# TencentEMapReduce/alluxio

Hardware: AMD Instinct MI355X
Metric: StressWorkerBench cached seq-read GB/s (whole node) at 1/2/4/8 MI355X workers (higher is better)
Workload: dtype uint8; 1 GPU; model=StressWorkerBench cached seq-read, HBM MEM tier, global_batch=256, seq_len=4096, parallelism=workers1, threads_per_worker=256, block_size=67108864, buffer_size=4096, page_size=2097152, verified=True, headline_verified=True, full=False

## Files before the change

### alluxio_amd/csrc/bindings.cpp

```cpp
#include <pybind11/pybind11.h>
#include <pybind11/stl.h>
#include <pybind11/numpy.h>

#include <cmath>
#include <cstring>
#include <vector>

#include "block_store.h"
#include "trace.h"
#include "cpu_codecs.h"
#include "ipc.h"
#include "numa_host.h"
#include "ring_read.h"
#include "ragged_gather.h"
#include "delim_index.h"
#include "field_parse.h"
#include "text_column.h"
#include "json_fields.h"
#include "parquet_decode.h"
#include "parquet_encode.h"
#include "parquet_stats.h"
#include "text_dict.h"
#include "kernels.h"
#include "seg_ring.h"
// ... 1144 lines not shown
          const size_t nc = (n + bpc - 1) / bpc;
          std::string out(nc * 4, '\0');
          {
            py::gil_scoped_release rel;
            for (size_t i = 0; i < nc; ++i) {
              const size_t off = i * bpc;
              const uint32_t c = crc32c_sw(p + off, std::min<size_t>(bpc, n - off), 0);
              out[4 * i] = char(c >> 24); out[4 * i + 1] = char(c >> 16);
              out[4 * i + 2] = char(c >> 8); out[4 * i + 3] = char(c);
            }
          }
          return py::bytes(out);
        }, py::arg("data"), py::arg("bytes_per_checksum") = 512);
  m.def("crc32c_combine", &crc32c_combine);
  m.def("crc32c_device_pages", &crc32c_device_pages, G(), py::arg("base"), py::arg("pages"), py::arg("length"),
        py::arg("page_bytes"));
  m.def("crc32c_device", &crc32c_device, G(), py::arg("ptr"), py::arg("length"), py::arg("piece") = 0,
        py::arg("stream") = 0);
  m.def("lz4_compress", [](py::bytes data) {
          std::string s = data;
          std::string out(lz4_compress_bound(s.size()), '\0');
          int64_t n;
          {
            py::gil_scoped_release rel;
            n = lz4_compress_block((const uint8_t*)s.data(), s.size(), (uint8_t*)&out[0], out.size());
          }
          if (n < 0) throw StoreError(kErrInvalidArgument, "lz4 compression failed");
          out.resize((size_t)n);
          return py::bytes(out);
        });
  m.def("lz4_decompress", [](py::bytes data, size_t capacity) {
          std::string s = data;
          std::string out(capacity, '\0');
          int64_t n;
          {
            py::gil_scoped_release rel;
            n = lz4_decompress_block((const uint8_t*)s.data(), s.size(), (uint8_t*)&out[0], out.size());
          }
          if (n < 0) throw StoreError(kErrInvalidArgument, "malformed lz4 block (" + std::to_string(n) + ")");
          out.resize((size_t)n);
          return py::bytes(out);
        });
  m.def("lz4_compress_bound", &lz4_compress_bound);
  m.def("trace_push", [](const std::string& name) { roctxRangePushA(name.c_str()); }, py::arg("name"));
  m.def("trace_pop", [] { roctxRangePop(); });
  m.def("trace_mark", [](const std::string& name) { roctxMarkA(name.c_str()); }, py::arg("name"));
  m.def("lz4_device", &lz4_device, G(), py::arg("chunks"), py::arg("compress"), py::arg("stream") = 0);
  m.def("lz4_device_kernel_ms", &lz4_device_kernel_ms, G(), py::arg("chunks"), py::arg("compress"),
        py::arg("reps") = 5);
  m.def("batched_copy", &batched_copy, G(), py::arg("segments"), py::arg("stream") = 0, py::arg("sync") = true);
  m.def("fill_pattern", [](uint64_t ptr, uint64_t bytes, uint64_t seed, uint64_t word_offset, uint64_t stream) {
          py::gil_scoped_release rel;
          HIP_CHECK(launch_fill_pattern(reinterpret_cast<uint8_t*>(ptr), bytes, seed, word_offset,
                                        reinterpret_cast<hipStream_t>(stream)));
        }, py::arg("ptr"), py::arg("bytes"), py::arg("seed"), py::arg("word_offset") = 0, py::arg("stream") = 0);
  m.def("store_fill", [](uint64_t ptr, uint64_t bytes, uint32_t word, bool nontemporal, unsigned grid,
                         uint64_t stream) {
          py::gil_scoped_release rel;
          unsigned used = 0;
          HIP_CHECK(launch_store_fill(reinterpret_cast<uint8_t*>(ptr), bytes, word, nontemporal, grid, &used,
                                      reinterpret_cast<hipStream_t>(stream)));
          return used;
        }, py::arg("ptr"), py::arg("bytes"), py::arg("word") = 0, py::arg("nontemporal") = false,
        py::arg("grid") = 0, py::arg("stream") = 0);
  m.def("evict_select_device", &evict_select_device);
  m.def("page_alloc_device", &page_alloc_device);
  m.def("set_copy_variant", &set_copy_variant, py::arg("variant"), py::arg("grid_cap") = 0);
  m.def("copy_variant", [] {
    int v = 0;
    unsigned cap = 0;
    copy_variant(&v, &cap);
    return py::make_tuple(v, cap);
  });
  m.def("set_crc_variant", &set_crc_variant, py::arg("variant"));
  m.def("set_lz4_decode_variant", &set_lz4_decode_variant, py::arg("variant"));
  m.def("set_lz4_encode_variant", &set_lz4_encode_variant, py::arg("variant"));
  m.def("set_seq_read_variant", &set_seq_read_variant, py::arg("variant"), py::arg("grid_cap") = 0);
  m.def("seq_read_variant", [] {
    int v = 0;
    unsigned cap = 0;
    seq_read_variant(&v, &cap);
    return py::make_tuple(v, cap);
  });
  m.def("seq_read_last_launch", [] {
    const SeqReadLaunch l = seq_read_last_launch();
    return py::make_tuple(l.fast ? "fast" : "general", l.unroll, l.grid);
  });
  m.def("set_ragged_gather_variant", &set_ragged_gather_variant, py::arg("variant"), py::arg("chunk_shift") = 0);
  m.def("ragged_gather_chunk_shift", &ragged_gather_chunk_shift);
  m.def("set_delim_index_variant", &set_delim_index_variant, py::arg("variant"), py::arg("tile_shift") = 0);
  m.def("delim_index_tile_shift", &delim_index_tile_shift);
  m.def("delim_index_variant", &delim_index_variant);
  m.def("set_delim_quote_variant", &set_delim_quote_variant, py::arg("variant"));
  m.def("delim_quote_variant", &delim_quote_variant);
  m.def("set_field_parse_variant", &set_field_parse_variant, py::arg("variant"));
  m.def("field_parse_variant", &field_parse_variant);
  m.def("set_text_column_variant", &set_text_column_variant, py::arg("variant"));
  m.def("text_column_variant", &text_column_variant);
  m.def("set_json_fields_variant", &set_json_fields_variant, py::arg("variant"));
  m.def("json_fields_variant", &json_fields_variant);
  m.def("set_json_text_variant", &set_json_text_variant, py::arg("variant"));
  m.def("json_text_variant", &json_text_variant);
  m.def("set_parquet_decode_variant", &set_parquet_decode_variant, py::arg("variant"));
  m.def("parquet_decode_variant", &parquet_decode_variant);
  m.def("set_text_dict_variant", &set_text_dict_variant, py::arg("variant"));
  m.def("text_dict_variant", &text_dict_variant);
  m.def("set_page_gather_chunk_variant", &set_page_gather_chunk_variant, py::arg("variant"));
  m.attr("COPY_CHUNK") = kCopyChunk;
}
```

### alluxio_amd/csrc/kernels.h

```cpp
#pragma once
#include <hip/hip_runtime.h>
#include <cstddef>
#include <cstdint>

#include "field_parse_host.h"
#include "json_fields_host.h"
#include "json_text_host.h"
#include "parquet_encode_host.h"
#include "parquet_host.h"
#include "parquet_stats_host.h"
#include "text_column_host.h"
#include "text_dict_host.h"

namespace amdx {

struct CopySeg {
  uint64_t src;
  uint64_t dst;
  uint64_t bytes;
  uint64_t chunk0;
};

constexpr uint64_t kCopyChunk = 256 * 1024;

hipError_t launch_batched_copy(const CopySeg* segs, int nseg, uint64_t total_chunks,
                               hipStream_t stream);
void set_copy_variant(int variant, unsigned grid_cap);
void copy_variant(int* variant, unsigned* grid_cap);

struct SeqReadArgs {
  const uint8_t* arena;
  const int64_t* ftab;
  const uint64_t* c_init;
  uint8_t* dst;
  uint64_t stream_stride;
  uint64_t file_len;
  uint64_t buf;
  uint64_t launch_base;
  uint32_t cycle;
  uint32_t streams;
  uint32_t depth;
  uint32_t page_shift;
  uint64_t footprint = 0;
  uint64_t base_mod = ~0ull;
};
constexpr uint32_t kSeqReadMaxStreams = 8192;
hipError_t launch_seq_read(const SeqReadArgs& a, hipStream_t stream);
void set_seq_read_variant(int variant, unsigned grid_cap);
void seq_read_variant(int* variant, unsigned* grid_cap);
struct SeqReadLaunch {
  int fast;
  int unroll;
  unsigned grid;
};
SeqReadLaunch seq_read_last_launch();
hipError_t launch_store_fill(uint8_t* dst, uint64_t bytes, uint32_t word, bool nontemporal, unsigned grid,
                             unsigned* grid_used, hipStream_t stream);

struct RaggedRow {
  uint64_t src;
  uint64_t dst_off;
  uint64_t span;
  uint32_t len;
  uint32_t chunk0;
};
struct RaggedRec {
  uint64_t start;
  uint32_t len;
  uint32_t pad;
};
struct RaggedGatherArgs {
  const uint8_t* arena;
  const int64_t* vtab;
  const RaggedRec* recs;
  const int64_t* idx;
  uint8_t* dst;
  uint64_t* out_off;
  uint32_t* out_len;
  RaggedRow* rows;
  uint32_t* chunk_pre;
  uint64_t n_rec;
  uint64_t row_stride;
  uint32_t batch;
  uint32_t page_shift;
  uint32_t align;
  uint32_t max_len;
  uint32_t padded;
  uint32_t pad_value;
  uint32_t total_chunks;
  uint32_t chunk_shift;
};
constexpr uint32_t kRaggedGatherMaxBatch = 65536;
hipError_t launch_ragged_gather(const RaggedGatherArgs& a, hipStream_t stream);
void set_ragged_gather_variant(int variant, unsigned chunk_shift);
uint32_t ragged_gather_chunk_shift();

struct DelimIndexArgs {
  const uint8_t* arena;
  const int64_t* vtab;
  uint32_t* tile_count;
  uint64_t* tile_base;
  uint64_t* out;
  uint64_t out_cap;
  uint64_t vstart;
  uint64_t bytes;
  uint64_t add;
  uint32_t ntiles;
  uint32_t page_shift;
  uint32_t tile_shift;
  uint32_t delim;
  uint32_t quote;
  uint32_t in_quote;
  uint32_t* tile_count_odd;
  uint32_t* tile_parity;
};
uint64_t delim_index_tiles(uint64_t vstart, uint64_t bytes, uint32_t tile_shift);
hipError_t launch_delim_count(const DelimIndexArgs& a, hipStream_t stream);
hipError_t launch_delim_scan(const DelimIndexArgs& a, hipStream_t stream);
hipError_t launch_delim_emit(const DelimIndexArgs& a, uint64_t total, hipStream_t stream);
hipError_t launch_delim_count_quoted(const DelimIndexArgs& a, hipStream_t stream);
hipError_t launch_delim_scan_quoted(const DelimIndexArgs& a, hipStream_t stream);
hipError_t launch_delim_emit_quoted(const DelimIndexArgs& a, uint64_t total, hipStream_t stream);
void set_delim_quote_variant(int variant);
int delim_quote_variant();
void set_delim_index_variant(int variant, unsigned tile_shift);
uint32_t delim_index_tile_shift();
int delim_index_variant();

hipError_t launch_field_parse(const FieldParseArgs& a, hipStream_t stream);
void set_field_parse_variant(int variant);
int field_parse_variant();

hipError_t launch_text_measure(const TextColumnArgs& a, hipStream_t stream);
hipError_t launch_text_emit(const TextColumnArgs& a, hipStream_t stream);
void set_text_column_variant(int variant);
int text_column_variant();
// ... 195 lines not shown
```

### alluxio_amd/csrc/kernels.hip

```cpp
#include "kernels.h"

#include <algorithm>
#include <cstring>
#include <mutex>

namespace amdx {

constexpr int kCopyThreads = 256;
typedef unsigned int u32x4 __attribute__((ext_vector_type(4)));

template <int P>
__device__ __forceinline__ u32x4 ld16(const u32x4* p) {
  if constexpr (P == 1) return __builtin_nontemporal_load(p);
  else return *p;
}
template <int P>
__device__ __forceinline__ void st16(u32x4* p, u32x4 v) {
  if constexpr (P == 1) __builtin_nontemporal_store(v, p);
  else *p = v;
}

__device__ __forceinline__ void copy_bytes(const uint8_t* __restrict__ s, uint8_t* __restrict__ d,
                                           uint64_t n, int tid) {
  for (uint64_t i = tid; i < n; i += kCopyThreads) d[i] = s[i];
// ... 68 lines not shown
  const dim3 block(kCopyThreads);
#define AMDX_COPY(U, L, S) hipLaunchKernelGGL((batched_copy_kernel<U, L, S>), grid, block, 0, stream, segs, nseg, total_chunks)
  switch (g_copy_variant) {
    case 1: AMDX_COPY(8, 0, 1); break;
    case 2: AMDX_COPY(8, 1, 0); break;
    case 3: AMDX_COPY(8, 1, 1); break;
    case 4: AMDX_COPY(4, 0, 0); break;
    case 5: AMDX_COPY(4, 0, 1); break;
    case 8: AMDX_COPY(16, 0, 0); break;
    case 9: AMDX_COPY(16, 0, 1); break;
    default: AMDX_COPY(8, 0, 0); break;
  }
#undef AMDX_COPY
  return hipGetLastError();
}

constexpr int kSeqThreads = 256;
constexpr uint32_t kSeqChunkShift = 10;
constexpr uint32_t kSeqChunk = 1u << kSeqChunkShift;

template <bool POW2, int UNROLL, int SP, int LP>
__global__ __launch_bounds__(kSeqThreads) void seq_read_kernel(SeqReadArgs a, uint32_t vpr_shift,
                                                               uint32_t depth_shift) {
  extern __shared__ uint32_t c0[];
  for (uint32_t s = threadIdx.x; s < a.streams; s += kSeqThreads)
    c0[s] = (uint32_t)((a.c_init[s] + a.launch_base) % a.cycle);
  __syncthreads();
  const uint64_t vpr = a.buf >> 4;
  const uint64_t nvec = (uint64_t)a.streams * a.depth * vpr;
  const uint64_t pmask = (1ull << a.page_shift) - 1;
  const uint64_t gstride = (uint64_t)gridDim.x * kSeqThreads;
  for (uint64_t base = (uint64_t)blockIdx.x * kSeqThreads + threadIdx.x; base < nvec;
       base += gstride * UNROLL) {
    u32x4 v[UNROLL];
    uint8_t* d[UNROLL];
    uint32_t nb[UNROLL];
#pragma unroll
    for (int u = 0; u < UNROLL; ++u) {
      const uint64_t i = base + (uint64_t)u * gstride;
      nb[u] = 0;
      d[u] = nullptr;
      if (i >= nvec) continue;
      uint64_t r, vi;
      uint32_t s, k;
      if constexpr (POW2) {
        r = i >> vpr_shift;
        vi = i & (vpr - 1);
        s = (uint32_t)(r >> depth_shift);
        k = (uint32_t)(r & (a.depth - 1));
      } else {
        r = i / vpr;
        vi = i - r * vpr;
        s = (uint32_t)(r / a.depth);
        k = (uint32_t)(r - (uint64_t)s * a.depth);
      }
      uint32_t c = c0[s] + k;
      if (c >= a.cycle) c = (uint32_t)(((uint64_t)c0[s] + k) % a.cycle);
      if (c == a.cycle - 1) continue;
      const uint64_t off = (uint64_t)c * a.buf + vi * 16;
      const uint64_t rend = ((uint64_t)c + 1) * a.buf;
      const uint64_t end = rend < a.file_len ? rend : a.file_len;
      if (off >= end) continue;
      const uint64_t page = (uint64_t)a.ftab[off >> a.page_shift];
      const uint8_t* src = a.arena + (page << a.page_shift) + (off & pmask);
      d[u] = a.dst + (uint64_t)s * a.stream_stride + (uint64_t)k * a.buf + vi * 16;
      if (end - off >= 16) {
        nb[u] = 16;
        v[u] = ld16<LP>(reinterpret_cast<const u32x4*>(src));
      } else {
        nb[u] = (uint32_t)(end - off);
        for (uint32_t b = 0; b < nb[u]; ++b) {
          const uint64_t o = off + b;
          d[u][b] = a.arena[((uint64_t)a.ftab[o >> a.page_shift] << a.page_shift) + (o & pmask)];
        }
      }
    }
#pragma unroll
    for (int u = 0; u < UNROLL; ++u)
      if (nb[u] == 16) st16<SP>(reinterpret_cast<u32x4*>(d[u]), v[u]);
  }
}

template <bool POW2>
__device__ __forceinline__ void seq_split(const SeqReadArgs& a, uint64_t q, uint64_t cpr, uint32_t cpr_shift,
                                          uint32_t depth_shift, uint32_t* s, uint32_t* k, uint64_t* ci) {
  if constexpr (POW2) {
    const uint64_t rd = q >> cpr_shift;
    *ci = q & (cpr - 1);
    *s = (uint32_t)(rd >> depth_shift);
    *k = (uint32_t)(rd & (a.depth - 1));
  } else {
    const uint64_t rd = q / cpr;
    *ci = q - rd * cpr;
    *s = (uint32_t)(rd / a.depth);
    *k = (uint32_t)(rd - (uint64_t)*s * a.depth);
  }
}

template <bool MULTI>
__device__ __forceinline__ uint64_t seq_call_index(const SeqReadArgs& a, uint64_t c0, uint32_t k) {
  if constexpr (MULTI) k %= a.cycle;
  uint64_t c = c0 + a.base_mod;
  c = c >= a.cycle ? c - a.cycle : c;
  c += k;
  return c >= a.cycle ? c - a.cycle : c;
}

template <bool POW2, int U, int SP, int LP, bool MULTI>
__device__ __forceinline__ void seq_fast_loop(const SeqReadArgs& a, const uint8_t* __restrict__ arena,
                                              const int64_t* __restrict__ ftab,
                                              const uint64_t* __restrict__ c_init, uint8_t* __restrict__ dst,
                                              uint32_t cpr_shift, uint32_t depth_shift) {
  constexpr uint32_t kWaves = kSeqThreads / 64;
  constexpr uint64_t kTrip = (uint64_t)U * kSeqChunk;
  constexpr int kGen = 4;
  const uint32_t lane16 = (threadIdx.x & 63u) * 16u;
  const uint32_t wave = (uint32_t)__builtin_amdgcn_readfirstlane((int)(threadIdx.x >> 6));
  const uint64_t cpr = a.buf >> kSeqChunkShift;
  const uint64_t per_stream = (uint64_t)a.depth * cpr;
  const uint64_t nchunks = (uint64_t)a.streams * per_stream;
  const uint64_t ngroups = (nchunks + U - 1) / U;
  const uint64_t nwaves = (uint64_t)gridDim.x * kWaves;
  const uint64_t pmask = (1ull << a.page_shift) - 1;
  for (uint64_t g = (uint64_t)blockIdx.x * kWaves + wave; g < ngroups; g += nwaves) {
    uint32_t s0, k0;
    uint64_t ci0;
    seq_split<POW2>(a, g * U, cpr, cpr_shift, depth_shift, &s0, &k0, &ci0);
    const uint64_t w0 = (uint64_t)k0 * cpr + ci0;
    const uint64_t off0 = seq_call_index<MULTI>(a, c_init[s0], k0) * a.buf + (ci0 << kSeqChunkShift);
    u32x4 v[U];
    if (w0 + U <= per_stream && off0 + kTrip <= a.file_len && (off0 & pmask) + kTrip <= pmask + 1) {
      const uint64_t page = (uint64_t)ftab[off0 >> a.page_shift];
      const u32x4* sp = reinterpret_cast<const u32x4*>(arena + (page << a.page_shift) + (off0 & pmask) + lane16);
      u32x4* dp = reinterpret_cast<u32x4*>(dst + (uint64_t)s0 * a.stream_stride + (w0 << kSeqChunkShift) + lane16);
#pragma unroll
      for (int u = 0; u < U; ++u) v[u] = ld16<LP>(sp + u * (kSeqChunk / 16));
#pragma unroll
      for (int u = 0; u < U; ++u) st16<SP>(dp + u * (kSeqChunk / 16), v[u]);
      continue;
    }
#pragma unroll 1
    for (int h = 0; h < U; h += kGen) {
      uint64_t dof[kGen], c0[kGen], sof[kGen];
      uint32_t k[kGen], n[kGen];
      int64_t page[kGen];
#pragma unroll
      for (int u = 0; u < kGen; ++u) {
        const uint64_t q = g * U + h + u;
        n[u] = q < nchunks ? kSeqChunk : 0;
        uint32_t s;
        uint64_t ci;
        seq_split<POW2>(a, q < nchunks ? q : 0, cpr, cpr_shift, depth_shift, &s, &k[u], &ci);
        sof[u] = ci << kSeqChunkShift;
        dof[u] = (uint64_t)s * a.stream_stride + (uint64_t)k[u] * a.buf + sof[u];
        c0[u] = c_init[s];
      }
#pragma unroll
      for (int u = 0; u < kGen; ++u) {
        const uint64_t c = seq_call_index<MULTI>(a, c0[u], k[u]);
        const uint64_t off = c * a.buf + sof[u];
        const bool data = c != a.cycle - 1 && off < a.file_len;
        const uint64_t left = data ? a.file_len - off : 0;
        n[u] = left < n[u] ? (uint32_t)left : n[u];
        sof[u] = data ? off : 0;
        page[u] = ftab[sof[u] >> a.page_shift];
      }
#pragma unroll
      for (int u = 0; u < kGen; ++u) {
        const uint8_t* src = arena + ((uint64_t)page[u] << a.page_shift) + (sof[u] & pmask);
        sof[u] = reinterpret_cast<uint64_t>(src);
        if (lane16 + 16 <= n[u]) v[u] = ld16<LP>(reinterpret_cast<const u32x4*>(src + lane16));
      }
#pragma unroll
      for (int u = 0; u < kGen; ++u) {
        if (lane16 + 16 <= n[u]) {
          st16<SP>(reinterpret_cast<u32x4*>(dst + dof[u] + lane16), v[u]);
        } else if (lane16 < n[u]) {
          const uint8_t* src = reinterpret_cast<const uint8_t*>(sof[u]);
          for (uint32_t b = lane16; b < n[u]; ++b) dst[dof[u] + b] = src[b];
        }
      }
    }
  }
}

template <bool POW2, int U, int SP, int LP>
__global__ __launch_bounds__(kSeqThreads) void seq_read_fast_kernel(
    SeqReadArgs a, const uint8_t* __restrict__ arena, const int64_t* __restrict__ ftab,
    const uint64_t* __restrict__ c_init, uint8_t* __restrict__ dst, uint32_t cpr_shift, uint32_t depth_shift) {
  if (a.depth > a.cycle) seq_fast_loop<POW2, U, SP, LP, true>(a, arena, ftab, c_init, dst, cpr_shift, depth_shift);
  else seq_fast_loop<POW2, U, SP, LP, false>(a, arena, ftab, c_init, dst, cpr_shift, depth_shift);
}

static int g_seq_variant = -1;
static unsigned g_seq_grid_cap = 8192;

void set_seq_read_variant(int variant, unsigned grid_cap) {
  g_seq_variant = variant;
  if (grid_cap) g_seq_grid_cap = grid_cap;
}
void seq_read_variant(int* variant, unsigned* grid_cap) {
  *variant = g_seq_variant;
  *grid_cap = g_seq_grid_cap;
}

static SeqReadLaunch g_seq_last;

SeqReadLaunch seq_read_last_launch() { return g_seq_last; }

static inline bool is_pow2(uint64_t x) { return x && !(x & (x - 1)); }
static inline uint32_t log2u(uint64_t x) {
  uint32_t s = 0;
  while ((1ull << s) < x) ++s;
  return s;
}

constexpr int kMaxDev = 64;
template <typename K>
static hipError_t resident_workgroups(K kernel, unsigned (&cached)[kMaxDev], unsigned* out) {
  static std::mutex mu;
  int dev = 0;
  hipError_t e = hipGetDevice(&dev);
  if (e != hipSuccess) return e;
  if (dev < 0 || dev >= kMaxDev) return hipErrorInvalidDevice;
  std::lock_guard<std::mutex> lk(mu);
  if (!cached[dev]) {
    int cus = 0, per_cu = 0;
    if ((e = hipDeviceGetAttribute(&cus, hipDeviceAttributeMultiprocessorCount, dev)) != hipSuccess) return e;
    if ((e = hipOccupancyMaxActiveBlocksPerMultiprocessor(&per_cu, kernel, kSeqThreads, 0)) != hipSuccess) return e;
    if (cus < 1 || per_cu < 1) return hipErrorInvalidValue;
    cached[dev] = (unsigned)cus * (unsigned)per_cu;
  }
  *out = cached[dev];
  return hipSuccess;
}

template <bool P2, int U, int SP, int LP>
static hipError_t seq_fast_resident(unsigned* out) {
  static unsigned cached[kMaxDev] = {};
  return resident_workgroups(seq_read_fast_kernel<P2, U, SP, LP>, cached, out);
}

template <bool P2, int U, int SP, int LP>
static hipError_t launch_seq_fast(const SeqReadArgs& a, hipStream_t stream) {
  unsigned resident = 0;
  const hipError_t e = seq_fast_resident<P2, U, SP, LP>(&resident);
  if (e != hipSuccess) return e;
  const uint64_t cpr = a.buf >> kSeqChunkShift;
  const uint64_t nchunks = (uint64_t)a.streams * a.depth * cpr;
  const uint64_t ngroups = (nchunks + U - 1) / U;
  constexpr uint64_t kWaves = kSeqThreads / 64;
  uint64_t blocks = (ngroups + kWaves - 1) / kWaves;
  if (blocks > resident) blocks = resident;
  if (blocks > g_seq_grid_cap) blocks = g_seq_grid_cap;
  if (blocks < 1) blocks = 1;
  hipLaunchKernelGGL((seq_read_fast_kernel<P2, U, SP, LP>), dim3((unsigned)blocks), dim3(kSeqThreads), 0, stream,
                     a, a.arena, a.ftab, a.c_init, a.dst, log2u(cpr), log2u(a.depth));
  g_seq_last = SeqReadLaunch{1, U, (unsigned)blocks};
  return hipGetLastError();
}

hipError_t launch_seq_read(const SeqReadArgs& a, hipStream_t stream) {
  if (a.streams == 0 || a.depth == 0 || a.buf == 0 || a.file_len == 0) return hipSuccess;
  if (a.streams > kSeqReadMaxStreams || (a.buf & 15) || (a.stream_stride & 15) ||
      ((uint64_t)a.dst & 15) || ((uint64_t)a.arena & 15))
    return hipErrorInvalidValue;
  const uint64_t vpr = a.buf >> 4;
  const uint64_t nvec = (uint64_t)a.streams * a.depth * vpr;
  const uint64_t fp = a.footprint ? a.footprint : a.file_len;
  const int var = g_seq_variant >= 0 ? g_seq_variant : (fp >= (128ull << 20) ? 4 : 0);
  const int unroll = (var & 2) ? 16 : 8;
  if ((a.buf & (kSeqChunk - 1)) == 0 && a.page_shift >= kSeqChunkShift && a.base_mod < a.cycle) {
    const bool p2 = is_pow2(a.buf >> kSeqChunkShift) && is_pow2(a.depth);
    const int sel = (p2 ? 8 : 0) | (unroll == 16 ? 4 : 0) | ((var & 1) ? 2 : 0) | ((var & 4) ? 1 : 0);
    switch (sel) {
#define AMDX_FAST(N, P2, U, SP, LP) case N: return launch_seq_fast<P2, U, SP, LP>(a, stream)
      AMDX_FAST(0, false, 8, 0, 0); AMDX_FAST(1, false, 8, 0, 1); AMDX_FAST(2, false, 8, 1, 0);
      AMDX_FAST(3, false, 8, 1, 1); AMDX_FAST(4, false, 16, 0, 0); AMDX_FAST(5, false, 16, 0, 1);
      AMDX_FAST(6, false, 16, 1, 0); AMDX_FAST(7, false, 16, 1, 1); AMDX_FAST(8, true, 8, 0, 0);
      AMDX_FAST(9, true, 8, 0, 1); AMDX_FAST(10, true, 8, 1, 0); AMDX_FAST(11, true, 8, 1, 1);
      AMDX_FAST(12, true, 16, 0, 0); AMDX_FAST(13, true, 16, 0, 1); AMDX_FAST(14, true, 16, 1, 0);
      default: AMDX_FAST(15, true, 16, 1, 1);
#undef AMDX_FAST
    }
  }
  uint64_t blocks = (nvec + (uint64_t)kSeqThreads * unroll - 1) / ((uint64_t)kSeqThreads * unroll);
  if (blocks > g_seq_grid_cap) blocks = g_seq_grid_cap;
  if (blocks < 1) blocks = 1;
  const bool p2 = is_pow2(vpr) && is_pow2(a.depth);
  const uint32_t vs = log2u(vpr), ds = log2u(a.depth);
  const size_t lds = a.streams * sizeof(uint32_t);
  const dim3 g((unsigned)blocks), b(kSeqThreads);
#define AMDX_SEQ(P2, U, SP, LP) \
  hipLaunchKernelGGL((seq_read_kernel<P2, U, SP, LP>), g, b, lds, stream, a, vs, ds)
  const int sp = var & 1, lp = (var >> 2) & 1;
  if (p2) {
    if (unroll == 16) {
      if (lp) { if (sp) AMDX_SEQ(true, 16, 1, 1); else AMDX_SEQ(true, 16, 0, 1); }
      else { if (sp) AMDX_SEQ(true, 16, 1, 0); else AMDX_SEQ(true, 16, 0, 0); }
    } else {
      if (lp) { if (sp) AMDX_SEQ(true, 8, 1, 1); else AMDX_SEQ(true, 8, 0, 1); }
      else { if (sp) AMDX_SEQ(true, 8, 1, 0); else AMDX_SEQ(true, 8, 0, 0); }
    }
  } else {
    if (lp) { if (sp) AMDX_SEQ(false, 8, 1, 1); else AMDX_SEQ(false, 8, 0, 1); }
    else { if (sp) AMDX_SEQ(false, 8, 1, 0); else AMDX_SEQ(false, 8, 0, 0); }
  }
#undef AMDX_SEQ
  g_seq_last = SeqReadLaunch{0, p2 ? unroll : 8, (unsigned)blocks};
  return hipGetLastError();
}

template <int SP>
__global__ __launch_bounds__(kSeqThreads) void store_fill_kernel(u32x4* __restrict__ dst, uint64_t nvec,
                                                                 uint32_t word) {
  constexpr uint32_t kWaves = kSeqThreads / 64;
  constexpr uint64_t kTripVec = 8 * (kSeqChunk / 16);
  const u32x4 v = {word, word, word, word};
  const uint32_t lane = threadIdx.x & 63u;
  const uint32_t wave = (uint32_t)__builtin_amdgcn_readfirstlane((int)(threadIdx.x >> 6));
  const uint64_t trips = nvec / kTripVec;
  const uint64_t nwaves = (uint64_t)gridDim.x * kWaves;
  for (uint64_t g = (uint64_t)blockIdx.x * kWaves + wave; g < trips; g += nwaves) {
    u32x4* p = dst + g * kTripVec + lane;
#pragma unroll
    for (int u = 0; u < 8; ++u) st16<SP>(p + u * (kSeqChunk / 16), v);
  }
  for (uint64_t i = trips * kTripVec + (uint64_t)blockIdx.x * kSeqThreads + threadIdx.x; i < nvec;
       i += (uint64_t)gridDim.x * kSeqThreads)
    st16<SP>(dst + i, v);
}

hipError_t launch_store_fill(uint8_t* dst, uint64_t bytes, uint32_t word, bool nontemporal, unsigned grid,
                             unsigned* grid_used, hipStream_t stream) {
  if (((uint64_t)dst & 15) || (bytes & 15)) return hipErrorInvalidValue;
  if (grid_used) *grid_used = 0;
  if (bytes == 0) return hipSuccess;
  static unsigned cached[2][kMaxDev] = {};
  unsigned resident = 0;
  const hipError_t e = nontemporal ? resident_workgroups(store_fill_kernel<1>, cached[1], &resident)
                                   : resident_workgroups(store_fill_kernel<0>, cached[0], &resident);
  if (e != hipSuccess) return e;
  const uint64_t nvec = bytes >> 4;
  uint64_t blocks = grid ? grid : resident;
  const uint64_t need = (nvec + kSeqThreads - 1) / kSeqThreads;
  if (blocks > need) blocks = need;
  if (nontemporal)
    hipLaunchKernelGGL(store_fill_kernel<1>, dim3((unsigned)blocks), dim3(kSeqThreads), 0, stream,
                       reinterpret_cast<u32x4*>(dst), nvec, word);
  else
    hipLaunchKernelGGL(store_fill_kernel<0>, dim3((unsigned)blocks), dim3(kSeqThreads), 0, stream,
                       reinterpret_cast<u32x4*>(dst), nvec, word);
  if (grid_used) *grid_used = (unsigned)blocks;
  return hipGetLastError();
}

constexpr uint32_t kCrcPoly = 0x82F63B78u;
constexpr uint64_t kCrcSeg = 64 * 1024;
constexpr int kCrcThreads = 256;
constexpr uint64_t kCrcLane = kCrcSeg / kCrcThreads;

__constant__ uint32_t c_crc_tab[8][256];
__constant__ uint32_t c_x2n[64];
__constant__ uint32_t c_crc16[16][256];
__constant__ uint32_t c_shift4k[4][256];
__constant__ uint32_t c_lane_shift[256];
constexpr int kCrc4Threads = 1024;
__constant__ uint32_t c_crc11[12][2048];
__constant__ uint32_t c_shift16k[4][256];
__constant__ uint32_t c_lane_shift1k[kCrc4Threads];
constexpr int kCrc5Threads = 1024;
constexpr uint64_t kCrc5Chunk = 64;
__constant__ uint32_t c_shift5[4][256];
__constant__ uint32_t c_lane_shift5[kCrc5Threads];

static void host_crc_tables(uint32_t tab[8][256], uint32_t x2n[64]) {
  for (uint32_t i = 0; i < 256; ++i) {
    uint32_t c = i;
    for (int k = 0; k < 8; ++k) c = (c & 1) ? (c >> 1) ^ kCrcPoly : c >> 1;
    tab[0][i] = c;
  }
  for (int t = 1; t < 8; ++t)
    for (uint32_t i = 0; i < 256; ++i) tab[t][i] = (tab[t - 1][i] >> 8) ^ tab[0][tab[t - 1][i] & 0xFF];
  auto mult = [](uint32_t a, uint32_t b) {
    uint32_t m = 1u << 31, p = 0;
    for (;;) {
      if (a & m) { p ^= b; if ((a & (m - 1)) == 0) break; }
      m >>= 1;
      b = (b & 1) ? (b >> 1) ^ kCrcPoly : b >> 1;
    }
    return p;
  };
// ... 2567 lines not shown
```

### alluxio_amd/csrc/ring_read.cpp

```cpp
#include "ring_read.h"

#include <algorithm>
#include <cstring>
#include <string>

#include "kernels.h"

namespace amdx {

RingReadSession::RingReadSession(BlockStore* store, int64_t session, const std::vector<int64_t>& block_ids,
                                 const std::vector<uint64_t>& block_lens, uint64_t dst_base,
                                 uint64_t stream_stride, uint64_t buf_bytes, uint32_t depth, uint32_t streams,
                                 int dst_kind, const std::vector<uint64_t>& start_offsets)
    : store_(store), session_(session), blocks_(block_ids), pins_(store), buf_(buf_bytes), stride_(stream_stride),
      dst_(dst_base), depth_(depth), streams_(streams), kind_(dst_kind) {
  if (block_ids.size() != block_lens.size() || block_ids.empty())
    throw StoreError(kErrInvalidArgument, "ring read: bad block list");
  for (uint64_t l : block_lens) file_len_ += l;
  check_shape();
  view_.append_file(store_, pins_, session_, blocks_, block_lens, "ring read");
  on_device_ = store_->has_device();
  finish_init(start_offsets);
}

RingReadSession::RingReadSession(uint64_t arena_base, const std::vector<int64_t>& file_pages, uint64_t page_size,
                                 uint64_t file_len, int device, uint64_t dst_base, uint64_t stream_stride,
                                 uint64_t buf_bytes, uint32_t depth, uint32_t streams, int dst_kind,
                                 const std::vector<uint64_t>& start_offsets)
    : store_(nullptr), session_(0), pins_(nullptr), file_len_(file_len), buf_(buf_bytes), stride_(stream_stride),
      dst_(dst_base), depth_(depth), streams_(streams), kind_(dst_kind), on_device_(device >= 0), device_(device) {
  check_shape();
  view_ = PagedView::raw(arena_base, file_pages, page_size, device, "ring read");
  if (view_.vtab.size() < (file_len_ + page_size - 1) / page_size)
    throw StoreError(kErrInvalidArgument, "ring read: page table shorter than the file");
  finish_init(start_offsets);
}

void RingReadSession::check_shape() {
  if (buf_ == 0 || depth_ == 0 || streams_ == 0 || streams_ > kSeqReadMaxStreams)
    throw StoreError(kErrInvalidArgument, "ring read: bad buffer/depth/stream count");
  if (stride_ < (uint64_t)depth_ * buf_) throw StoreError(kErrInvalidArgument, "ring read: stride too small");
  if (file_len_ == 0) throw StoreError(kErrInvalidArgument, "ring read: empty file");
  const uint64_t calls = (file_len_ + buf_ - 1) / buf_;
  if (calls + 1 >= (1ull << 32)) throw StoreError(kErrInvalidArgument, "ring read: too many calls per pass");
  cycle_ = (uint32_t)(calls + 1);
  full_passes_ = depth_ / cycle_;
  rem_calls_ = depth_ % cycle_;
}

void RingReadSession::set_device() const {
  if (store_) store_->use_device();
  else if (device_ >= 0) AMDX_HIP(hipSetDevice(device_));
}

void RingReadSession::finish_init(const std::vector<uint64_t>& start_offsets) {
  c_init_.assign(streams_, 0);
  for (uint32_t s = 0; s < streams_ && s < start_offsets.size(); ++s) {
    if (start_offsets[s] % buf_) throw StoreError(kErrInvalidArgument, "ring read: start offsets must be buffer aligned");
    c_init_[s] = std::min<uint64_t>(start_offsets[s] / buf_, cycle_ - 1);
  }
  std::vector<uint64_t> starts(c_init_);
  std::sort(starts.begin(), starts.end());
  const uint64_t distinct = (uint64_t)(std::unique(starts.begin(), starts.end()) - starts.begin());
  footprint_ = std::min<uint64_t>(file_len_, distinct * depth_ * buf_);
  lockstep_ = distinct == 1;
  if (on_device_) {
    if (buf_ & 15 || stride_ & 15 || dst_ & 15)
      throw StoreError(kErrInvalidArgument, "ring read: buffer size, stride and ring base must be 16-byte aligned");
    set_device();
    d_ftab_.alloc(view_.vtab.size() * sizeof(int64_t));
    d_cinit_.alloc(c_init_.size() * sizeof(uint64_t));
    AMDX_HIP(hipMemcpy(d_ftab_.p, view_.vtab.data(), view_.vtab.size() * sizeof(int64_t), hipMemcpyHostToDevice));
    AMDX_HIP(hipMemcpy(d_cinit_.p, c_init_.data(), c_init_.size() * sizeof(uint64_t), hipMemcpyHostToDevice));
  }
}

RingReadSession::~RingReadSession() {
  try {
    close();
  } catch (...) {
  }
}

void RingReadSession::close() {
  if (closed_) return;
  closed_ = true;
  d_ftab_.reset();
  d_cinit_.reset();
  pins_.release();
}

uint64_t RingReadSession::step_bytes(uint64_t c0, uint64_t* eofs) const {
  auto before = [this](uint64_t x) {
    return x < cycle_ ? std::min<uint64_t>(x * buf_, file_len_)
                      : file_len_ + std::min<uint64_t>((x - cycle_) * buf_, file_len_);
  };
  const uint64_t c1 = c0 + rem_calls_;
  *eofs = (uint64_t)full_passes_ + (c1 >= cycle_ ? 1 : 0);
  return (uint64_t)full_passes_ * file_len_ + before(c1) - before(c0);
}

uint64_t RingReadSession::step(uint64_t stream, uint64_t* eofs) {
  if (closed_) throw StoreError(kErrInvalidState, "ring read session closed");
  const uint64_t base = calls_per_stream_;
  if (on_device_) {
    set_device();
    SeqReadArgs a;
    a.arena = view_.base();
    a.ftab = d_ftab_.as<int64_t>();
    a.c_init = d_cinit_.as<uint64_t>();
    a.dst = reinterpret_cast<uint8_t*>(dst_);
    a.stream_stride = stride_;
    a.file_len = file_len_;
    a.buf = buf_;
    a.launch_base = base;
    a.base_mod = base_mod_;
    a.cycle = cycle_;
    a.streams = streams_;
    a.depth = depth_;
    a.page_shift = view_.page_shift;
    a.footprint = footprint_;
    hipStream_t st = reinterpret_cast<hipStream_t>(stream);
    AMDX_HIP(launch_seq_read(a, st));
    if (kind_ == (int)MemKind::kHost) AMDX_HIP(hipStreamSynchronize(st));
  } else {
    for (uint32_t s = 0; s < streams_; ++s)
      for (uint32_t k = 0; k < depth_; ++k) {
        auto [off, len] = std::pair<uint64_t, uint64_t>(0, 0);
        const uint64_t c = (c_init_[s] + base_mod_ + k) % cycle_;
        if (c == cycle_ - 1) continue;
        off = c * buf_;
        len = std::min(buf_, file_len_ - off);
        uint8_t* d = reinterpret_cast<uint8_t*>(dst_ + s * stride_ + (uint64_t)k * buf_);
        for_each_page_run(view_.base(), view_.vtab.data(), view_.page_shift, off, len,
                          [d](const uint8_t* p, uint64_t n, uint64_t done) { std::memcpy(d + done, p, n); });
      }
  }
  auto first_call = [this](uint32_t s) {
    const uint64_t c = c_init_[s] + base_mod_;
    return c >= cycle_ ? c - cycle_ : c;
  };
  uint64_t bytes = 0, eof = 0;
  if (lockstep_) {
    bytes = step_bytes(first_call(0), &eof) * streams_;
    eof *= streams_;
  } else {
    for (uint32_t s = 0; s < streams_; ++s) {
      uint64_t e = 0;
      bytes += step_bytes(first_call(s), &e);
      eof += e;
    }
  }
  calls_per_stream_ += depth_;
  base_mod_ += rem_calls_;
  if (base_mod_ >= cycle_) base_mod_ -= cycle_;
  total_ += bytes;
  reopens_ += eof;
  if (store_) store_->access_blocks(blocks_);
  if (eofs) *eofs = eof;
  return bytes;
}

uint64_t RingReadSession::position(uint32_t s) const {
  const uint64_t c = (c_init_.at(s) + calls_per_stream_) % cycle_;
  return std::min<uint64_t>(c * buf_, file_len_);
}

std::pair<uint64_t, uint64_t> RingReadSession::last_call(uint32_t s, uint32_t k) const {
  if (calls_per_stream_ < depth_) return {0, 0};
  const uint64_t c = (c_init_.at(s) + calls_per_stream_ - depth_ + k) % cycle_;
  if (c == cycle_ - 1) return {file_len_, 0};
  const uint64_t off = c * buf_;
  return {off, std::min(buf_, file_len_ - off)};
}

}
```

### alluxio_amd/csrc/ring_read.h

```cpp
#pragma once
#include <cstdint>
#include <vector>

#include "paged_view.h"

namespace amdx {

class RingReadSession {
 public:
  RingReadSession(BlockStore* store, int64_t session, const std::vector<int64_t>& block_ids,
                  const std::vector<uint64_t>& block_lens, uint64_t dst_base, uint64_t stream_stride,
                  uint64_t buf_bytes, uint32_t depth, uint32_t streams, int dst_kind,
                  const std::vector<uint64_t>& start_offsets);
  RingReadSession(uint64_t arena_base, const std::vector<int64_t>& file_pages, uint64_t page_size,
                  uint64_t file_len, int device, uint64_t dst_base, uint64_t stream_stride, uint64_t buf_bytes,
                  uint32_t depth, uint32_t streams, int dst_kind, const std::vector<uint64_t>& start_offsets);
  ~RingReadSession();
  uint64_t step(uint64_t stream, uint64_t* eofs);
  void close();
  uint64_t total_bytes() const { return total_; }
  uint64_t reopens() const { return reopens_; }
  uint64_t calls() const { return calls_per_stream_; }
  uint64_t position(uint32_t s) const;
  std::pair<uint64_t, uint64_t> last_call(uint32_t s, uint32_t k) const;
  uint64_t file_len() const { return file_len_; }

 private:
  uint64_t step_bytes(uint64_t c0, uint64_t* eofs) const;
  void check_shape();
  void finish_init(const std::vector<uint64_t>& start_offsets);
  void set_device() const;
  BlockStore* store_;
  int64_t session_;
  std::vector<int64_t> blocks_;
  BlockPins pins_;
  uint64_t file_len_ = 0, buf_, stride_, dst_;
  uint32_t depth_, streams_, cycle_;
  int kind_;
  bool on_device_ = false;
  int device_ = -1;
  PagedView view_;
  std::vector<uint64_t> c_init_;
  uint64_t footprint_ = 0;
  bool lockstep_ = false;
  uint32_t full_passes_ = 0, rem_calls_ = 0;
  uint64_t base_mod_ = 0;
  DevBuf d_ftab_, d_cinit_;
  uint64_t calls_per_stream_ = 0, total_ = 0, reopens_ = 0;
  bool closed_ = false;
};

}
```

Before: 6509 GB/s.

## Cache seq-read launch plan and inline cursor/page table into kernel args

```diff
diff --git a/alluxio_amd/csrc/bindings.cpp b/alluxio_amd/csrc/bindings.cpp
--- a/alluxio_amd/csrc/bindings.cpp
+++ b/alluxio_amd/csrc/bindings.cpp
@@ -1250,10 +1250,12 @@
     seq_read_variant(&v, &cap);
     return py::make_tuple(v, cap);
   });
-  m.def("seq_read_last_launch", [] {
+  m.def("seq_read_last_launch", [](bool detail) -> py::tuple {
     const SeqReadLaunch l = seq_read_last_launch();
+    if (detail)
+      return py::make_tuple(l.fast ? "fast" : "general", l.unroll, l.grid, l.cursor_inline != 0, l.pages_inline);
     return py::make_tuple(l.fast ? "fast" : "general", l.unroll, l.grid);
-  });
+  }, py::arg("detail") = false);
   m.def("set_ragged_gather_variant", &set_ragged_gather_variant, py::arg("variant"), py::arg("chunk_shift") = 0);
   m.def("ragged_gather_chunk_shift", &ragged_gather_chunk_shift);
   m.def("set_delim_index_variant", &set_delim_index_variant, py::arg("variant"), py::arg("tile_shift") = 0);
diff --git a/alluxio_amd/csrc/kernels.h b/alluxio_amd/csrc/kernels.h
--- a/alluxio_amd/csrc/kernels.h
+++ b/alluxio_amd/csrc/kernels.h
@@ -28,6 +28,7 @@
 void set_copy_variant(int variant, unsigned grid_cap);
 void copy_variant(int* variant, unsigned* grid_cap);
 
+constexpr uint32_t kSeqInlinePages = 4;
 struct SeqReadArgs {
   const uint8_t* arena;
   const int64_t* ftab;
@@ -43,15 +44,33 @@
   uint32_t page_shift;
   uint64_t footprint = 0;
   uint64_t base_mod = ~0ull;
+  uint64_t c_uniform = 0;
+  uint32_t cursor_set = 0;
+  uint32_t page_n = 0;
+  uint32_t page_first = 0;
+  uint32_t file_pages = 0;
+  uint32_t page_tab[kSeqInlinePages] = {};
 };
 constexpr uint32_t kSeqReadMaxStreams = 8192;
 hipError_t launch_seq_read(const SeqReadArgs& a, hipStream_t stream);
+struct SeqReadPlan {
+  const void* kernel = nullptr;
+  uint32_t epoch = 0;
+  uint32_t grid = 0;
+  uint32_t cpr_shift = 0, depth_shift = 0;
+  int unroll = 0;
+};
+uint32_t seq_read_epoch();
+hipError_t plan_seq_read(const SeqReadArgs& a, SeqReadPlan* plan);
+hipError_t launch_seq_plan(const SeqReadPlan& plan, const SeqReadArgs& a, hipStream_t stream);
 void set_seq_read_variant(int variant, unsigned grid_cap);
 void seq_read_variant(int* variant, unsigned* grid_cap);
 struct SeqReadLaunch {
   int fast;
   int unroll;
   unsigned grid;
+  int cursor_inline;
+  unsigned pages_inline;
 };
 SeqReadLaunch seq_read_last_launch();
 hipError_t launch_store_fill(uint8_t* dst, uint64_t bytes, uint32_t word, bool nontemporal, unsigned grid,
diff --git a/alluxio_amd/csrc/kernels.hip b/alluxio_amd/csrc/kernels.hip
--- a/alluxio_amd/csrc/kernels.hip
+++ b/alluxio_amd/csrc/kernels.hip
@@ -174,28 +174,43 @@
 }
 
 template <bool POW2>
-__device__ __forceinline__ void seq_split(const SeqReadArgs& a, uint64_t q, uint64_t cpr, uint32_t cpr_shift,
-                                          uint32_t depth_shift, uint32_t* s, uint32_t* k, uint64_t* ci) {
+__device__ __forceinline__ void seq_split(const SeqReadArgs& a, uint32_t q, uint32_t cpr, uint32_t cpr_shift,
+                                          uint32_t depth_shift, uint32_t* s, uint32_t* k, uint32_t* ci) {
   if constexpr (POW2) {
-    const uint64_t rd = q >> cpr_shift;
+    const uint32_t rd = q >> cpr_shift;
     *ci = q & (cpr - 1);
-    *s = (uint32_t)(rd >> depth_shift);
-    *k = (uint32_t)(rd & (a.depth - 1));
+    *s = rd >> depth_shift;
+    *k = rd & (a.depth - 1);
   } else {
-    const uint64_t rd = q / cpr;
+    const uint32_t rd = q / cpr;
     *ci = q - rd * cpr;
-    *s = (uint32_t)(rd / a.depth);
-    *k = (uint32_t)(rd - (uint64_t)*s * a.depth);
-  }
+    *s = rd / a.depth;
+    *k = rd - *s * a.depth;
+  }
+}
+
+__device__ __forceinline__ uint32_t seq_first_call(const SeqReadArgs& a, uint32_t c0) {
+  const uint32_t room = a.cycle - (uint32_t)a.base_mod;
+  return c0 >= room ? c0 - room : c0 + (uint32_t)a.base_mod;
 }
 
 template <bool MULTI>
-__device__ __forceinline__ uint64_t seq_call_index(const SeqReadArgs& a, uint64_t c0, uint32_t k) {
+__device__ __forceinline__ uint32_t seq_call_index(const SeqReadArgs& a, uint32_t first, uint32_t k) {
   if constexpr (MULTI) k %= a.cycle;
-  uint64_t c = c0 + a.base_mod;
-  c = c >= a.cycle ? c - a.cycle : c;
-  c += k;
-  return c >= a.cycle ? c - a.cycle : c;
+  const uint32_t room = a.cycle - first;
+  return k >= room ? k - room : first + k;
+}
+
+__device__ __forceinline__ uint64_t seq_page(const SeqReadArgs& a, uint32_t e0, uint32_t e1, uint32_t e2, uint32_t e3,
+                                             const int64_t* __restrict__ ftab, uint32_t page) {
+  static_assert(kSeqInlinePages == 4, "one register and one select per inline entry");
+  const uint32_t d = page >= a.page_first ? page - a.page_first : page + (a.file_pages - a.page_first);
+  if (d >= a.page_n) return (uint64_t)ftab[page];
+  uint32_t e = e0;
+  e = d == 1 ? e1 : e;
+  e = d == 2 ? e2 : e;
+  e = d == 3 ? e3 : e;
+  return e;
 }
 
 template <bool POW2, int U, int SP, int LP, bool MULTI>
@@ -204,27 +219,33 @@
                                               const uint64_t* __restrict__ c_init, uint8_t* __restrict__ dst,
                                               uint32_t cpr_shift, uint32_t depth_shift) {
   constexpr uint32_t kWaves = kSeqThreads / 64;
-  constexpr uint64_t kTrip = (uint64_t)U * kSeqChunk;
-  constexpr int kGen = 4;
+  constexpr int kGen = 2;
   const uint32_t lane16 = (threadIdx.x & 63u) * 16u;
   const uint32_t wave = (uint32_t)__builtin_amdgcn_readfirstlane((int)(threadIdx.x >> 6));
-  const uint64_t cpr = a.buf >> kSeqChunkShift;
-  const uint64_t per_stream = (uint64_t)a.depth * cpr;
-  const uint64_t nchunks = (uint64_t)a.streams * per_stream;
-  const uint64_t ngroups = (nchunks + U - 1) / U;
-  const uint64_t nwaves = (uint64_t)gridDim.x * kWaves;
-  const uint64_t pmask = (1ull << a.page_shift) - 1;
-  for (uint64_t g = (uint64_t)blockIdx.x * kWaves + wave; g < ngroups; g += nwaves) {
-    uint32_t s0, k0;
-    uint64_t ci0;
+  const uint32_t cpr = (uint32_t)(a.buf >> kSeqChunkShift);
+  const uint32_t per_stream = a.depth * cpr;
+  const uint32_t nchunks = a.streams * per_stream;
+  const uint32_t ngroups = (nchunks + U - 1) / U;
+  const uint32_t nwaves = gridDim.x * kWaves;
+  const uint32_t file_chunks = (uint32_t)(a.file_len >> kSeqChunkShift);
+  const uint32_t pc_shift = a.page_shift - kSeqChunkShift;
+  const uint32_t pcmask = (1u << pc_shift) - 1;
+  const uint32_t first_shared = seq_first_call(a, (uint32_t)a.c_uniform);
+  uint32_t e0 = a.page_tab[0], e1 = a.page_tab[1], e2 = a.page_tab[2], e3 = a.page_tab[3];
+  asm volatile("" : "+s"(e0), "+s"(e1), "+s"(e2), "+s"(e3));
+  for (uint32_t g = blockIdx.x * kWaves + wave; g < ngroups; g += nwaves) {
+    uint32_t s0, k0, ci0;
     seq_split<POW2>(a, g * U, cpr, cpr_shift, depth_shift, &s0, &k0, &ci0);
-    const uint64_t w0 = (uint64_t)k0 * cpr + ci0;
-    const uint64_t off0 = seq_call_index<MULTI>(a, c_init[s0], k0) * a.buf + (ci0 << kSeqChunkShift);
-    u32x4 v[U];
-    if (w0 + U <= per_stream && off0 + kTrip <= a.file_len && (off0 & pmask) + kTrip <= pmask + 1) {
-      const uint64_t page = (uint64_t)ftab[off0 >> a.page_shift];
-      const u32x4* sp = reinterpret_cast<const u32x4*>(arena + (page << a.page_shift) + (off0 & pmask) + lane16);
-      u32x4* dp = reinterpret_cast<u32x4*>(dst + (uint64_t)s0 * a.stream_stride + (w0 << kSeqChunkShift) + lane16);
+    const uint32_t w0 = k0 * cpr + ci0;
+    const uint32_t first = a.cursor_set ? first_shared : seq_first_call(a, (uint32_t)c_init[s0]);
+    const uint32_t f0 = seq_call_index<MULTI>(a, first, k0) * cpr + ci0;
+    if (w0 + U <= per_stream && f0 + U <= file_chunks && (f0 & pcmask) + U <= pcmask + 1) {
+      const uint64_t page = seq_page(a, e0, e1, e2, e3, ftab, f0 >> pc_shift);
+      const u32x4* sp = reinterpret_cast<const u32x4*>(
+          arena + (page << a.page_shift) + ((uint64_t)(f0 & pcmask) << kSeqChunkShift) + lane16);
+      u32x4* dp = reinterpret_cast<u32x4*>(dst + (uint64_t)s0 * a.stream_stride +
+                                           ((uint64_t)w0 << kSeqChunkShift) + lane16);
+      u32x4 v[U];
 #pragma unroll
       for (int u = 0; u < U; ++u) v[u] = ld16<LP>(sp + u * (kSeqChunk / 16));
 #pragma unroll
@@ -233,40 +254,40 @@
     }
 #pragma unroll 1
     for (int h = 0; h < U; h += kGen) {
-      uint64_t dof[kGen], c0[kGen], sof[kGen];
-      uint32_t k[kGen], n[kGen];
-      int64_t page[kGen];
+      uint64_t dof[kGen], sof[kGen];
+      uint32_t c0[kGen], k[kGen], ci[kGen], n[kGen];
+      uint64_t page[kGen];
+      u32x4 w[kGen] = {};
 #pragma unroll
       for (int u = 0; u < kGen; ++u) {
-        const uint64_t q = g * U + h + u;
+        const uint32_t q = g * U + h + u;
         n[u] = q < nchunks ? kSeqChunk : 0;
         uint32_t s;
-        uint64_t ci;
-        seq_split<POW2>(a, q < nchunks ? q : 0, cpr, cpr_shift, depth_shift, &s, &k[u], &ci);
-        sof[u] = ci << kSeqChunkShift;
-        dof[u] = (uint64_t)s * a.stream_stride + (uint64_t)k[u] * a.buf + sof[u];
-        c0[u] = c_init[s];
+        seq_split<POW2>(a, q < nchunks ? q : 0, cpr, cpr_shift, depth_shift, &s, &k[u], &ci[u]);
+        dof[u] = (uint64_t)s * a.stream_stride + ((uint64_t)(k[u] * cpr + ci[u]) << kSeqChunkShift);
+        c0[u] = a.cursor_set ? (uint32_t)a.c_uniform : (uint32_t)c_init[s];
       }
 #pragma unroll
       for (int u = 0; u < kGen; ++u) {
-        const uint64_t c = seq_call_index<MULTI>(a, c0[u], k[u]);
-        const uint64_t off = c * a.buf + sof[u];
+        const uint32_t c = seq_call_index<MULTI>(a, seq_first_call(a, c0[u]), k[u]);
+        const uint32_t f = c * cpr + ci[u];
+        const uint64_t off = (uint64_t)f << kSeqChunkShift;
         const bool data = c != a.cycle - 1 && off < a.file_len;
         const uint64_t left = data ? a.file_len - off : 0;
         n[u] = left < n[u] ? (uint32_t)left : n[u];
         sof[u] = data ? off : 0;
-        page[u] = ftab[sof[u] >> a.page_shift];
+        page[u] = (uint64_t)ftab[sof[u] >> a.page_shift];
       }
 #pragma unroll
       for (int u = 0; u < kGen; ++u) {
-        const uint8_t* src = arena + ((uint64_t)page[u] << a.page_shift) + (sof[u] & pmask);
+        const uint8_t* src = arena + (page[u] << a.page_shift) + (sof[u] & ((1ull << a.page_shift) - 1));
         sof[u] = reinterpret_cast<uint64_t>(src);
-        if (lane16 + 16 <= n[u]) v[u] = ld16<LP>(reinterpret_cast<const u32x4*>(src + lane16));
+        if (lane16 + 16 <= n[u]) w[u] = ld16<LP>(reinterpret_cast<const u32x4*>(src + lane16));
       }
 #pragma unroll
       for (int u = 0; u < kGen; ++u) {
         if (lane16 + 16 <= n[u]) {
-          st16<SP>(reinterpret_cast<u32x4*>(dst + dof[u] + lane16), v[u]);
+          st16<SP>(reinterpret_cast<u32x4*>(dst + dof[u] + lane16), w[u]);
         } else if (lane16 < n[u]) {
           const uint8_t* src = reinterpret_cast<const uint8_t*>(sof[u]);
           for (uint32_t b = lane16; b < n[u]; ++b) dst[dof[u] + b] = src[b];
@@ -287,14 +308,18 @@
 static int g_seq_variant = -1;
 static unsigned g_seq_grid_cap = 8192;
 
+static uint32_t g_seq_epoch = 1;
+
 void set_seq_read_variant(int variant, unsigned grid_cap) {
   g_seq_variant = variant;
   if (grid_cap) g_seq_grid_cap = grid_cap;
+  if (++g_seq_epoch == 0) g_seq_epoch = 1;
 }
 void seq_read_variant(int* variant, unsigned* grid_cap) {
   *variant = g_seq_variant;
   *grid_cap = g_seq_grid_cap;
 }
+uint32_t seq_read_epoch() { return g_seq_epoch; }
 
 static SeqReadLaunch g_seq_last;
 
@@ -327,16 +352,14 @@
   return hipSuccess;
 }
 
+using SeqFastKernel = void (*)(SeqReadArgs, const uint8_t*, const int64_t*, const uint64_t*, uint8_t*, uint32_t,
+                               uint32_t);
+
 template <bool P2, int U, int SP, int LP>
-static hipError_t seq_fast_resident(unsigned* out) {
+static hipError_t plan_seq_fast(const SeqReadArgs& a, SeqReadPlan* plan) {
   static unsigned cached[kMaxDev] = {};
-  return resident_workgroups(seq_read_fast_kernel<P2, U, SP, LP>, cached, out);
-}
-
-template <bool P2, int U, int SP, int LP>
-static hipError_t launch_seq_fast(const SeqReadArgs& a, hipStream_t stream) {
   unsigned resident = 0;
-  const hipError_t e = seq_fast_resident<P2, U, SP, LP>(&resident);
+  const hipError_t e = resident_workgroups(seq_read_fast_kernel<P2, U, SP, LP>, cached, &resident);
   if (e != hipSuccess) return e;
   const uint64_t cpr = a.buf >> kSeqChunkShift;
   const uint64_t nchunks = (uint64_t)a.streams * a.depth * cpr;
@@ -346,36 +369,82 @@
   if (blocks > resident) blocks = resident;
   if (blocks > g_seq_grid_cap) blocks = g_seq_grid_cap;
   if (blocks < 1) blocks = 1;
-  hipLaunchKernelGGL((seq_read_fast_kernel<P2, U, SP, LP>), dim3((unsigned)blocks), dim3(kSeqThreads), 0, stream,
-                     a, a.arena, a.ftab, a.c_init, a.dst, log2u(cpr), log2u(a.depth));
-  g_seq_last = SeqReadLaunch{1, U, (unsigned)blocks};
+  plan->kernel = reinterpret_cast<const void*>(static_cast<SeqFastKernel>(seq_read_fast_kernel<P2, U, SP, LP>));
+  plan->grid = (uint32_t)blocks;
+  plan->cpr_shift = log2u(cpr);
+  plan->depth_shift = log2u(a.depth);
+  plan->unroll = U;
+  return hipSuccess;
+}
+
+static bool seq_args_ok(const SeqReadArgs& a) {
+  return !(a.streams > kSeqReadMaxStreams || (a.buf & 15) || (a.stream_stride & 15) || ((uint64_t)a.dst & 15) ||
+           ((uint64_t)a.arena & 15));
+}
+static bool seq_args_empty(const SeqReadArgs& a) {
+  return a.streams == 0 || a.depth == 0 || a.buf == 0 || a.file_len == 0;
+}
+static int seq_variant_of(const SeqReadArgs& a) {
+  const uint64_t fp = a.footprint ? a.footprint : a.file_len;
+  return g_seq_variant >= 0 ? g_seq_variant : (fp >= (128ull << 20) ? 4 : 0);
+}
+
+static bool seq_fast_shape(const SeqReadArgs& a) {
+  if ((a.buf & (kSeqChunk - 1)) || a.page_shift < kSeqChunkShift || a.page_shift > 40 || a.base_mod >= a.cycle)
+    return false;
+  const uint64_t cpr = a.buf >> kSeqChunkShift, lim = (1ull << 32) - 16;
+  if (cpr >= (1ull << 31)) return false;
+  const uint64_t per_stream = (uint64_t)a.depth * cpr;
+  return per_stream < lim && (uint64_t)a.streams * per_stream < lim && (uint64_t)a.cycle * cpr < lim;
+}
+
+hipError_t plan_seq_read(const SeqReadArgs& a, SeqReadPlan* plan) {
+  *plan = SeqReadPlan{};
+  plan->epoch = g_seq_epoch;
+  if (seq_args_empty(a)) return hipSuccess;
+  if (!seq_args_ok(a)) return hipErrorInvalidValue;
+  if (!seq_fast_shape(a)) return hipSuccess;
+  const int var = seq_variant_of(a);
+  const bool p2 = is_pow2(a.buf >> kSeqChunkShift) && is_pow2(a.depth);
+  const int sel = (p2 ? 8 : 0) | ((var & 2) ? 4 : 0) | ((var & 1) ? 2 : 0) | ((var & 4) ? 1 : 0);
+  switch (sel) {
+#define AMDX_FAST(N, P2, U, SP, LP) case N: return plan_seq_fast<P2, U, SP, LP>(a, plan)
+    AMDX_FAST(0, false, 8, 0, 0); AMDX_FAST(1, false, 8, 0, 1); AMDX_FAST(2, false, 8, 1, 0);
+    AMDX_FAST(3, false, 8, 1, 1); AMDX_FAST(4, false, 16, 0, 0); AMDX_FAST(5, false, 16, 0, 1);
+    AMDX_FAST(6, false, 16, 1, 0); AMDX_FAST(7, false, 16, 1, 1); AMDX_FAST(8, true, 8, 0, 0);
+    AMDX_FAST(9, true, 8, 0, 1); AMDX_FAST(10, true, 8, 1, 0); AMDX_FAST(11, true, 8, 1, 1);
+    AMDX_FAST(12, true, 16, 0, 0); AMDX_FAST(13, true, 16, 0, 1); AMDX_FAST(14, true, 16, 1, 0);
+    default: AMDX_FAST(15, true, 16, 1, 1);
+#undef AMDX_FAST
+  }
+}
+
+static hipError_t launch_seq_general(const SeqReadArgs& a, hipStream_t stream);
+
+hipError_t launch_seq_plan(const SeqReadPlan& plan, const SeqReadArgs& a, hipStream_t stream) {
+  if (seq_args_empty(a)) return hipSuccess;
+  if (!plan.kernel) return seq_args_ok(a) ? launch_seq_general(a, stream) : hipErrorInvalidValue;
+  if (a.base_mod >= a.cycle || a.page_n > kSeqInlinePages || (a.cursor_set && a.c_uniform >= a.cycle) ||
+      (a.page_n && (a.file_pages == 0 || a.page_first >= a.file_pages)))
+    return hipErrorInvalidValue;
+  hipLaunchKernelGGL(reinterpret_cast<SeqFastKernel>(const_cast<void*>(plan.kernel)), dim3(plan.grid),
+                     dim3(kSeqThreads), 0, stream, a, a.arena, a.ftab, a.c_init, a.dst, plan.cpr_shift,
+                     plan.depth_shift);
+  g_seq_last = SeqReadLaunch{1, plan.unroll, plan.grid, a.cursor_set ? 1 : 0, a.page_n};
   return hipGetLastError();
 }
 
 hipError_t launch_seq_read(const SeqReadArgs& a, hipStream_t stream) {
-  if (a.streams == 0 || a.depth == 0 || a.buf == 0 || a.file_len == 0) return hipSuccess;
-  if (a.streams > kSeqReadMaxStreams || (a.buf & 15) || (a.stream_stride & 15) ||
-      ((uint64_t)a.dst & 15) || ((uint64_t)a.arena & 15))
-    return hipErrorInvalidValue;
+  SeqReadPlan plan;
+  const hipError_t e = plan_seq_read(a, &plan);
+  return e != hipSuccess ? e : launch_seq_plan(plan, a, stream);
+}
+
+static hipError_t launch_seq_general(const SeqReadArgs& a, hipStream_t stream) {
   const uint64_t vpr = a.buf >> 4;
   const uint64_t nvec = (uint64_t)a.streams * a.depth * vpr;
-  const uint64_t fp = a.footprint ? a.footprint : a.file_len;
-  const int var = g_seq_variant >= 0 ? g_seq_variant : (fp >= (128ull << 20) ? 4 : 0);
+  const int var = seq_variant_of(a);
   const int unroll = (var & 2) ? 16 : 8;
-  if ((a.buf & (kSeqChunk - 1)) == 0 && a.page_shift >= kSeqChunkShift && a.base_mod < a.cycle) {
-    const bool p2 = is_pow2(a.buf >> kSeqChunkShift) && is_pow2(a.depth);
-    const int sel = (p2 ? 8 : 0) | (unroll == 16 ? 4 : 0) | ((var & 1) ? 2 : 0) | ((var & 4) ? 1 : 0);
-    switch (sel) {
-#define AMDX_FAST(N, P2, U, SP, LP) case N: return launch_seq_fast<P2, U, SP, LP>(a, stream)
-      AMDX_FAST(0, false, 8, 0, 0); AMDX_FAST(1, false, 8, 0, 1); AMDX_FAST(2, false, 8, 1, 0);
-      AMDX_FAST(3, false, 8, 1, 1); AMDX_FAST(4, false, 16, 0, 0); AMDX_FAST(5, false, 16, 0, 1);
-      AMDX_FAST(6, false, 16, 1, 0); AMDX_FAST(7, false, 16, 1, 1); AMDX_FAST(8, true, 8, 0, 0);
-      AMDX_FAST(9, true, 8, 0, 1); AMDX_FAST(10, true, 8, 1, 0); AMDX_FAST(11, true, 8, 1, 1);
-      AMDX_FAST(12, true, 16, 0, 0); AMDX_FAST(13, true, 16, 0, 1); AMDX_FAST(14, true, 16, 1, 0);
-      default: AMDX_FAST(15, true, 16, 1, 1);
-#undef AMDX_FAST
-    }
-  }
   uint64_t blocks = (nvec + (uint64_t)kSeqThreads * unroll - 1) / ((uint64_t)kSeqThreads * unroll);
   if (blocks > g_seq_grid_cap) blocks = g_seq_grid_cap;
   if (blocks < 1) blocks = 1;
@@ -399,7 +468,7 @@
     else { if (sp) AMDX_SEQ(false, 8, 1, 0); else AMDX_SEQ(false, 8, 0, 0); }
   }
 #undef AMDX_SEQ
-  g_seq_last = SeqReadLaunch{0, p2 ? unroll : 8, (unsigned)blocks};
+  g_seq_last = SeqReadLaunch{0, p2 ? unroll : 8, (unsigned)blocks, 0, 0};
   return hipGetLastError();
 }
 
diff --git a/alluxio_amd/csrc/ring_read.cpp b/alluxio_amd/csrc/ring_read.cpp
--- a/alluxio_amd/csrc/ring_read.cpp
+++ b/alluxio_amd/csrc/ring_read.cpp
@@ -64,6 +64,13 @@
   const uint64_t distinct = (uint64_t)(std::unique(starts.begin(), starts.end()) - starts.begin());
   footprint_ = std::min<uint64_t>(file_len_, distinct * depth_ * buf_);
   lockstep_ = distinct == 1;
+  const uint64_t pages = (file_len_ + (1ull << view_.page_shift) - 1) >> view_.page_shift;
+  bool fit = pages < (1ull << 32) && pages <= view_.vtab.size();
+  for (uint64_t p = 0; fit && p < pages; ++p) fit = view_.vtab[p] >= 0 && view_.vtab[p] < (int64_t)(1ull << 32);
+  if (fit) {
+    file_pages_ = (uint32_t)pages;
+    inline_pages_ = kSeqInlinePages;
+  }
   if (on_device_) {
     if (buf_ & 15 || stride_ & 15 || dst_ & 15)
       throw StoreError(kErrInvalidArgument, "ring read: buffer size, stride and ring base must be 16-byte aligned");
@@ -120,8 +127,21 @@
     a.depth = depth_;
     a.page_shift = view_.page_shift;
     a.footprint = footprint_;
+    a.cursor_set = lockstep_;
+    a.c_uniform = c_init_[0];
+    uint64_t first = c_init_[0] + base_mod_;
+    if (first >= cycle_) first -= cycle_;
+    uint64_t page = first == cycle_ - 1 ? 0 : (first * buf_) >> view_.page_shift;
+    a.page_first = (uint32_t)page;
+    a.file_pages = file_pages_;
+    a.page_n = inline_pages_;
+    for (uint32_t i = 0; i < inline_pages_; ++i) {
+      a.page_tab[i] = (uint32_t)view_.vtab[page];
+      if (++page == file_pages_) page = 0;
+    }
     hipStream_t st = reinterpret_cast<hipStream_t>(stream);
-    AMDX_HIP(launch_seq_read(a, st));
+    if (plan_.epoch != seq_read_epoch()) AMDX_HIP(plan_seq_read(a, &plan_));
+    AMDX_HIP(launch_seq_plan(plan_, a, st));
     if (kind_ == (int)MemKind::kHost) AMDX_HIP(hipStreamSynchronize(st));
   } else {
     for (uint32_t s = 0; s < streams_; ++s)
diff --git a/alluxio_amd/csrc/ring_read.h b/alluxio_amd/csrc/ring_read.h
--- a/alluxio_amd/csrc/ring_read.h
+++ b/alluxio_amd/csrc/ring_read.h
@@ -2,6 +2,7 @@
 #include <cstdint>
 #include <vector>
 
+#include "kernels.h"
 #include "paged_view.h"
 
 namespace amdx {
@@ -45,6 +46,8 @@
   bool lockstep_ = false;
   uint32_t full_passes_ = 0, rem_calls_ = 0;
   uint64_t base_mod_ = 0;
+  uint32_t file_pages_ = 0, inline_pages_ = 0;
+  SeqReadPlan plan_;
   DevBuf d_ftab_, d_cinit_;
   uint64_t calls_per_stream_ = 0, total_ = 0, reopens_ = 0;
   bool closed_ = false;
```

Measured after the change: 6584 GB/s, median of 6. 1.2% higher.
